# ToyotaResearchInstitute/conex

Hardware: AMD Instinct MI355X
Metric: Newton KKT-solves/sec (assemble+factor+solve), 1000x(20x20) PSD blocks, fp64 (higher is better)
Workload: dtype f64

## Files before the change

### conex_amd/csrc/kkt_context.hip

```cpp
#include <hip/hip_ext.h>
#include "kkt_internal.h"
#include "kernels_cone.hip.h"
#include "kernels_gemm.hip.h"
#include "kernels_kkt_big.hip.h"
#include "kernels_oct.hip.h"
#include "kernels_lmi.hip.h"
#include "lmi_fused_mfma.h"
#include "kernels_lmi_sparse.hip.h"
#include "kernels_lmi_rows.hip.h"
#include "kernels_lmi_large.hip.h"
#include "kernels_quad.hip.h"


namespace cxk_host {

int Fail(cxk_context* ctx, const char* msg) {
  ctx->err = msg;
  fprintf(stderr, "conex_kkt_hip: %s\n", msg);
  return CXK_FAILURE;
}

bool IsUnique(int N, int m, const int* x) {
  std::vector<char> seen(N > 0 ? N : 1, 0);
  for (int i = 0; i < m; i++) {
// ... 889 lines not shown
    CXK_CHAIN(24, 0, 24, 0)
    CXK_CHAIN(24, 8, 24, 8)
    CXK_CHAIN(32, 16, 32, 16)
    CXK_CHAIN(8, 8, 24, 0)
    CXK_CHAIN(16, 8, 24, 0)
    CXK_CHAIN(8, 8, 16, 8)
    CXK_CHAIN(24, 0, 24, 8)
    CXK_CHAIN(24, 0, 32, 16)
#undef CXK_CHAIN
    CXK_DEMAND(done, "internal error: no tree_chain_lean instance for the chain's shapes");
    CXK_TRY(hipGetLastError());
  return CXK_SUCCESS;
}

int MakeFusedTreeArgs(cxk_context* ctx, FusedTreeArgs* out) {
  if (*ctx->fx_flag != 0.0) {
    CXK_TRY(hipStreamSynchronize(ctx->stream));
    CXK_TRY(hipMemcpy(ctx->fx_hand.p, ctx->fx_hand_init.data(), sizeof(double) * ctx->fx_hand_init.size(), hipMemcpyHostToDevice));
    unsigned long long bits = kFusedSentinel;
    double sent;
    memcpy(&sent, &bits, sizeof(sent));
    std::vector<double> ys(ctx->fx_ysig.n, sent);
    CXK_TRY(hipMemcpy(ctx->fx_ysig.p, ys.data(), sizeof(double) * ys.size(), hipMemcpyHostToDevice));
    if (ctx->fx_done.p) {
      CXK_TRY(hipMemset(ctx->fx_done.p, 0, sizeof(unsigned long long) * ctx->fx_done.n));
      ctx->fx_done_target = 0;
    }
    *ctx->fx_flag = 0.0;
    ctx->timeout_pending = true;
  }
  FusedTreeArgs& a = *out;
  a.rec = ctx->fx_rec.p;
  a.count = (int)ctx->level_sn.size();
  a.G = ctx->G.p;
  a.AWc = ctx->AWc.p;
  a.AQcc = ctx->AQcc.p;
  a.b = ctx->b.p;
  a.AW = ctx->AW.p;
  a.AQc = ctx->AQc.p;
  a.slab = ctx->slab.p;
  a.y = ctx->y.p;
  a.pub = ctx->fx_pub.p;
  a.tg_reg = ctx->tg_reg.p;
  a.xreg = ctx->fx_xreg.p;
  a.xsrc = ctx->fx_xsrc.p;
  a.rsrc = ctx->fx_rsrc.p;
// ... 13 lines not shown
  a.k_from = nullptr;
  a.comb = 0;
  a.form = 0;
  a.sc = ctx->sc.p;
  a.sys_sc = ctx->sys_sc.p;
  a.K = (int)ctx->cons.size();
  a.host_flag = ctx->fx_flag;
  a.up_sleep = 30;
  a.count_up = ctx->fused_shard ? ctx->fused_up : a.count;
  a.x = ctx->xbuf.p;
  a.n_xs = ctx->n_xs;
  a.n_xv = ctx->n_xv;
  a.xg = ctx->fx_xg.p;
  a.as_src = ctx->as_src.p;
  a.xs_pt = ctx->xs_pt.p;
  a.pt_ptr = ctx->pt_ptr.p;
  a.pt_src = ctx->pt_src.p;
  a.xr = ctx->fx_xr.p;
  a.rs_src = ctx->rs_src.p;
  a.pf_ptr = ctx->pf_ptr.p;
  a.pf_src = ctx->pf_src.p;
  a.done = ctx->fx_done.p;
  a.done_target = 0;
  return CXK_SUCCESS;
}

int ShardAllReduce(cxk_context* ctx, double* buf, size_t count, int op);
long ExchangeCount(const cxk_context* ctx);

void RaiseHostWord(void* flag) { *static_cast<double*>(flag) = 1.0; }
int DebugReportTimeout(cxk_context* ctx) {
  CXK_TRY(hipMemcpyAsync(ctx->d_fail.p + 1, &ctx->asm_tag, sizeof(int), hipMemcpyHostToDevice, ctx->stream));
  if (ctx->debug_stream_ordered) {
    CXK_TRY(hipLaunchHostFunc(ctx->stream, RaiseHostWord, ctx->fx_flag));
    return CXK_SUCCESS;
  }
  CXK_TRY(hipStreamSynchronize(ctx->stream));
  *ctx->fx_flag = 1.0;
  return CXK_SUCCESS;
}

int LaunchFusedShard(cxk_context* ctx) {
  const cxk_context::AsmPending ap = ctx->asm_pending;
  ctx->asm_pending.on = false;
  FusedTreeArgs a;
  if (MakeFusedTreeArgs(ctx, &a)) return CXK_FAILURE;
// ... 2244 lines not shown
    if (r > 0 || n == 1) total += ms;
  }
  if (avg_ms) *avg_ms = total / (n > 1 ? n - 1 : 1);
  CXK_TRY(hipMemcpy(C, dC.p, sizeof(double) * nc * batch, hipMemcpyDeviceToHost));
  (void)hipEventDestroy(e0);
  (void)hipEventDestroy(e1);
  return CXK_SUCCESS;
}

int cxk_dense_top_columns(const cxk_context* ctx) {
  if (!ctx || !ctx->finalized) return -1;
  return ctx->top_dense.on ? ctx->top_dense.args.T : 0;
}

int cxk_count_sparse_lmi(const cxk_context* ctx) {
  if (!ctx || !ctx->finalized) return -1;
  int k = 0;
  for (size_t i = 0; i < ctx->cons.size(); i++) k += ctx->cons[i].type == CXK_LMI && ctx->owned[i] && ctx->cons[i].sparse;
  return k;
}

int cxk_fused_assembly(const cxk_context* ctx) { return ctx && ctx->fused_asm ? 1 : 0; }
int cxk_fused_tree(const cxk_context* ctx) { return ctx && ctx->fused_tree ? 1 : 0; }

int cxk_fused_tree_timed_out(cxk_context* ctx) {
  if (!ctx || !ctx->timeout_unreported) return 0;
  ctx->timeout_unreported = false;
  return 1;
}

int cxk_debug_force_fused_timeout(cxk_context* ctx) {
  if (!ctx || !ctx->fx_flag || !ctx->fused_tree) return CXK_FAILURE;
  *ctx->fx_flag = 1.0;
  return CXK_SUCCESS;
}

int cxk_debug_fused_timeout_at(cxk_context* ctx, int launch_index, int which) {
  if (!ctx || !ctx->device_ready || !ctx->fx_flag || !ctx->fused_tree) return CXK_FAILURE;
  const bool stream_ordered = (which & CXK_DEBUG_FUSED_STREAM_ORDERED) != 0;
  which &= ~CXK_DEBUG_FUSED_STREAM_ORDERED;
  if (stream_ordered && which != CXK_DEBUG_FUSED_SHARD_TOP) return CXK_FAILURE;
  if (which != CXK_DEBUG_FUSED_FACTOR && which != CXK_DEBUG_FUSED_SHARD_UP && which != CXK_DEBUG_FUSED_SHARD_TOP)
    return CXK_FAILURE;
  if ((which == CXK_DEBUG_FUSED_FACTOR) != (ctx->world <= 1) || (ctx->world > 1 && !ctx->fused_shard))
    return CXK_FAILURE;
  ctx->debug_timeout_at = launch_index >= 0 ? ctx->fused_launches + launch_index : -1;
// ... 140 lines not shown
```

### conex_amd/csrc/kkt_internal.h

```cpp
#pragma once
#include <hip/hip_runtime.h>
#include <dlfcn.h>
#include <rccl/rccl.h>

#include <algorithm>
#include <atomic>
#include <cfloat>
#include <climits>
#include <cmath>
#include <cstdio>
#include <cstdlib>
#include <cstring>
#include <iterator>
#include <map>
#include <memory>
#include <string>
#include <tuple>
#include <vector>

#include "../../include/conex_kkt_hip.h"
#include "kernels_kkt.hip.h"
#include "kernels_kkt_top.hip.h"
#include "lmi_types.h"
#include "symbolic.h"
// ... 167 lines not shown
  DevBuf<int> rs_var2;
  int64_t as_T2 = 0;
  int rs_N2 = 0;
  struct AsmPending {
    bool on = false;
    int with_rhs = 0;
    double k = 0, bs = 0, cs = 0, cb = 0, cq = 0, cw = 0;
  } asm_pending;
  bool fused_tree = false;
  bool fused_split = false;
  bool fused_sweep = false;
  bool fused_shard = false;
  int fused_up = 0;
  DevBuf<GatherRec> fx_xg;
  DevBuf<ResidRec> fx_xr;
  DevBuf<unsigned long long> fx_done;
  unsigned long long fx_done_target = 0;
  int fused_sa = 0, fused_sb = 0;
  DevBuf<int> fx_rec, fx_xreg;
  DevBuf<long long> fx_xsrc, fx_rsrc;
  DevBuf<int> fx_pub;
  DevBuf<double> fx_hand, fx_ysig;
  std::vector<double> fx_hand_init;
  long long fx_updb_base = 0;
  long long fx_fwd_stride = 0;
  unsigned fused_tgen = 0;
  DevBuf<double> y3;
  bool y3_valid = false;
  double y3_bs = 0, y3_cs = 0;
  bool y_deferred = false;
  bool no_y_deferral = false;
  DevBuf<unsigned long long> y_done;
  unsigned long long y_done_target = 0;
  bool no_triple = false;
  unsigned fused_gen = 0;
  double* fx_flag = nullptr;
  int debug_timeout_at = -1, debug_timeout_site = 0, fused_launches = 0;
  int fused_timeouts = 0;
  bool timeout_pending = false;
  bool timeout_unreported = false;
  long long shard_settled_seq = -1;
  int shard_fused_tag = 0;
  long long collectives = 0, shard_launch_collectives = 0;
  bool debug_stream_ordered = false;
  long long calls = 0, redo_call = -1;
  bool asm_deferred = false;
// ... 94 lines not shown
```

### conex_amd/csrc/kkt_plans.hip

```cpp
#define CXK_DEVICE_FUNCTIONS_ONLY
#include "kkt_internal.h"
#include "big_chol.h"

namespace cxk_host {

void ComputeTreeStructure(cxk_context* ctx) {
  const Layout& L = ctx->lay;
  const int K = ctx->md.K;
  ctx->t_ns.assign(K, 0);
  ctx->t_nsep.assign(K, 0);
  ctx->t_start.assign(K, 0);
  ctx->t_level.assign(K, 0);
  ctx->t_parent.assign(K, -1);
  for (int e = 0; e < K; e++) {
    ctx->t_ns[e] = L.supernode_size[e];
    ctx->t_nsep[e] = (int)L.separators[e].size();
    ctx->t_start[e] = L.supernode_start[e];
    if (ctx->t_nsep[e] > 0) ctx->t_parent[e] = L.var_to_sn[L.separators[e][0]];
  }
  for (int i = 0; i < K; i++) {
    if (ctx->t_ns[i] == 0) continue;
    for (int v : L.separators[i]) {
      const int p = L.var_to_sn[v];
      if (ctx->t_level[p] < ctx->t_level[i] + 1) ctx->t_level[p] = ctx->t_level[i] + 1;
// ... 104 lines not shown
      const int64_t n = ctx->t_ns[e];
      ctx->n_xs += n * (n + 1) / 2 + n * ctx->t_nsep[e];
      ctx->n_xv += (int)n;
    }
}

namespace {

struct PlanSwitches {
  bool no_big_dataflow = getenv("CXK_NO_BIG_DATAFLOW") != nullptr;
  bool debug_levels = getenv("CXK_DEBUG_LEVELS") != nullptr;
  bool no_lean = getenv("CXK_NO_LEAN") != nullptr;
  bool no_ranges = getenv("CXK_NO_RANGES") != nullptr;
  bool keep_top = getenv("CXK_KEEP_TOP") != nullptr;
  bool no_chain = getenv("CXK_NO_CHAIN") != nullptr;
  bool no_back_pairs = getenv("CXK_NO_BACK_PAIRS") != nullptr;
  bool no_fused_asm = getenv("CXK_NO_FUSED_ASM") != nullptr;
  bool no_fused_shard = getenv("CXK_NO_FUSED_SHARD") != nullptr;
  bool no_fused_tree = getenv("CXK_NO_FUSED_TREE") != nullptr;
  bool no_fused_wide = getenv("CXK_NO_FUSED_WIDE") != nullptr;
  bool fused_split = getenv("CXK_FUSED_SPLIT") != nullptr;
  bool fused_level_order = getenv("CXK_FUSED_LEVEL_ORDER") != nullptr;
  bool no_fused_sweep = getenv("CXK_NO_FUSED_SWEEP") != nullptr;
  bool no_top_dense = getenv("CXK_NO_TOP_DENSE") != nullptr;
};

struct Verdict {
  bool ok = true;
  const char* why = nullptr;
  bool check(bool cond, const char* msg) {
    ok = ok && cond;
    if (!ok && !why) why = msg;
    return ok;
  }
  void note(const char* msg) { check(true, msg); }
  int refuse(const PlanSwitches& sw, const char* strategy) const {
    if (sw.debug_levels) fprintf(stderr, "%s not taken: %s\n", strategy, why ? why : "(unnamed check)");
    return CXK_SUCCESS;
  }
};

template <typename Rec>
std::vector<Rec> Flatten(const std::vector<std::vector<int64_t>>& lists, std::vector<int>* ptr, std::vector<int64_t>* src) {
  std::vector<Rec> recs(lists.size());
  ptr->assign(lists.size() + 1, 0);
  for (size_t t = 0; t < lists.size(); t++) {
// ... 714 lines not shown
  std::vector<int> v2;
  for (int pvar = 0; pvar < N; pvar++)
    if (!var_own[pvar]) {
      r2.push_back(rg.rec[pvar]);
      v2.push_back(pvar);
    }
  ctx->as_T2 = (int64_t)g2.size();
  ctx->rs_N2 = (int)v2.size();
  if (g2.empty()) g2.push_back(GatherRec{0, -1, 0, 0});
  if (v2.empty()) {
    r2.push_back(ResidRec{-1, 0, 0});
    v2.push_back(0);
  }
  CXK_TRY(ctx->asm_rec.upload(arecs));
  CXK_TRY(ctx->as_rec2.upload(g2));
  CXK_TRY(ctx->rs_rec2.upload(r2));
  CXK_TRY(ctx->rs_var2.upload(v2));
  ctx->fused_asm = true;
  return CXK_SUCCESS;
}


struct FusedTables {
  std::vector<int> recs, xreg, pub;
  std::vector<long long> xsrc, rsrc;
};

bool FusedTreeShapes(const cxk_context* ctx, const PlanSwitches& sw, const UpdateSlots& u, Verdict& v, int* sa, int* sb) {
  const int nlev = ctx->nlev;
  const std::vector<int>& ns = ctx->t_ns;
  const int cnt_all = (int)ctx->level_sn.size();
  const bool wide_single = v.ok && ctx->world <= 1 && cnt_all == 1 && ctx->md.K >= 1 && ns[ctx->level_sn[0]] > 32 &&
                           ns[ctx->level_sn[0]] <= 64 && ctx->t_nsep[ctx->level_sn[0]] == 0 && !sw.no_fused_wide;
  if (wide_single) {
    *sa = *sb = ((ns[ctx->level_sn[0]] + 7) / 8 * 8) << 8;
    return true;
  }
  std::vector<int> shapes;
  for (int l = 0; l < nlev && v.ok; l++) {
    if (ctx->level_ptr[l + 1] == ctx->level_ptr[l]) continue;
    v.ok = !ctx->level_big[l] && ctx->level_nh[l] == ctx->level_ptr[l + 1] - ctx->level_ptr[l];
    for (auto& sg : ctx->level_segs[l]) {
      v.ok = v.ok && sg.shape != 0 && sg.inl;
      if (std::find(shapes.begin(), shapes.end(), sg.shape) == shapes.end()) shapes.push_back(sg.shape);
    }
    for (int pos = ctx->level_ptr[l]; pos < ctx->level_ptr[l + 1] && v.ok; pos++) {
      const int e = ctx->level_sn[pos];
// ... 125 lines not shown
      }
    v.ok = ft->rsrc.size() < (size_t)INT32_MAX && ft->xreg.size() < (size_t)INT32_MAX;
  }
}

void FusedTreePublished(const cxk_context* ctx, const UpdateSlots& u, const std::vector<int>& pos_of, size_t n_upd,
                        size_t n_updb, Verdict& v, FusedTables* ft) {
  const Layout& L = ctx->lay;
  const int cnt_all = (int)ctx->level_sn.size();
  for (int pos = 0; pos < cnt_all && v.ok; pos++) {
    const int e = ctx->level_sn[pos];
    for (int x : L.separators[e]) v.check(pos_of[L.var_to_sn[x]] > pos, "a consumer at a lower position");
  }
  v.ok = v.ok && n_upd + n_updb + 8 < (size_t)INT32_MAX;
  for (int pos = 0; pos < cnt_all && v.ok; pos++) {
    const int e = ctx->level_sn[pos];
    const int nsep = ctx->t_nsep[e];
    int* w = ft->recs.data() + (size_t)pos * kFusedRecWords;
    w[21] = w[22] = 0;
    w[23] = (int)ft->pub.size();
    for (int64_t t = 0; t < (int64_t)nsep * (nsep + 1) / 2; t++) ft->pub.push_back(u.pub_dst[(size_t)(u.upd_off[e] + t)]);
    for (int c = 0; c < nsep; c++) ft->pub.push_back((int)n_upd + u.pubb_dst[(size_t)(u.updb_off[e] + c)]);
  }
}

void DealOverXcds(const cxk_context* ctx, const std::vector<int>& pos_of, std::vector<int>* recs) {
  const Layout& L = ctx->lay;
  const int cnt_all = (int)ctx->level_sn.size();
  std::vector<std::vector<int>> kids(cnt_all);
  std::vector<int> roots;
  for (int pos = 0; pos < cnt_all; pos++) {
    int par = INT32_MAX;
    for (int v : L.separators[ctx->level_sn[pos]]) par = std::min(par, pos_of[L.var_to_sn[v]]);
    if (par == INT32_MAX)
      roots.push_back(pos);
    else
      kids[par].push_back(pos);
  }
  std::vector<int> dfs, stack(roots.rbegin(), roots.rend());
  dfs.reserve(cnt_all);
  while (!stack.empty()) {
    const int u = stack.back();
    stack.pop_back();
    dfs.push_back(u);
    for (auto it = kids[u].rbegin(); it != kids[u].rend(); ++it) stack.push_back(*it);
  }
// ... 69 lines not shown
  if (!v.ok) return v.refuse(sw, "whole-tree launch");
  ft.xreg.resize(ft.xreg.size() + kPullPad, 0);
  ft.xsrc.resize(ft.xsrc.size() + kPullPad * kFusedExtraMax, -1ll);
  ft.rsrc.resize(ft.rsrc.size() + 64 * kFusedExtraMax, -1ll);
  ft.pub.resize(ft.pub.size() + 64, (int)u.slots);
  const double sent = [] {
    double d;
    const unsigned long long bits = kFusedSentinel;
    memcpy(&d, &bits, sizeof(d));
    return d;
  }();
  const size_t hs = us + 3 * ubs + 8;
  ctx->fx_updb_base = (long long)us;
  ctx->fx_fwd_stride = (long long)ubs;
  ctx->fx_hand_init.assign(2 * hs, 0.0);
  for (size_t t = 0; t + 64 < ft.pub.size(); t++) {
    const int d = ft.pub[t];
    if (d != (int)u.slots && d != (int)us + u.slotsb) {
      ctx->fx_hand_init[d] = ctx->fx_hand_init[hs + d] = sent;
      if ((size_t)d >= us)
        for (size_t q = 1; q < 3; q++) ctx->fx_hand_init[d + q * ubs] = ctx->fx_hand_init[hs + d + q * ubs] = sent;
    }
  }
  if (!split && !sharded && !sw.fused_level_order) DealOverXcds(ctx, pos_of, &ft.recs);
  CXK_TRY(ctx->fx_rec.upload(ft.recs));
  CXK_TRY(ctx->fx_xreg.upload(ft.xreg));
  CXK_TRY(ctx->fx_xsrc.upload(ft.xsrc));
  CXK_TRY(ctx->fx_rsrc.upload(ft.rsrc));
  CXK_TRY(ctx->fx_pub.upload(ft.pub));
  CXK_TRY(ctx->fx_hand.upload(ctx->fx_hand_init));
  CXK_TRY(ctx->fx_ysig.upload(std::vector<double>(6 * (size_t)N, sent)));
  CXK_TRY(ctx->y3.alloc(3 * (size_t)N, true));
  ctx->fused_tgen = 0;
  ctx->y3_valid = false;
  if (!ctx->fx_flag) {
    CXK_TRY(hipHostMalloc(reinterpret_cast<void**>(&ctx->fx_flag), 64, hipHostMallocDefault));
    *ctx->fx_flag = 0.0;
  }
  ctx->fused_sa = sa;
  ctx->fused_sb = sb;
  ctx->fused_gen = 0;
  ctx->fused_tree = true;
  ctx->fused_split = split;
  ctx->fused_shard = sharded;
  ctx->fused_up = cnt_up;
  ctx->fused_sweep = !sharded && !sw.no_fused_sweep;
  if (sw.debug_levels)
    fprintf(stderr, "whole tree in %s: %d supernodes, shapes <%d,%d> <%d,%d>, %zu entries / %zu variables with further sources\n",
            sharded ? "two launches around the exchange (own subtrees up + pack, top + down)" : split ? "two launches (up, down)" : "one launch", cnt_all, sa >> 8, sa & 255, sb >> 8, sb & 255,
            ft.xreg.size() - kPullPad, ft.rsrc.size());
  return CXK_SUCCESS;
}

int PlanTopDense(cxk_context* ctx, const PlanSwitches& sw, const UpdateSlots& u) {
  const Layout& L = ctx->lay;
  const int K = ctx->md.K, N = ctx->md.N, nlev = ctx->nlev;
  const std::vector<int>& ns = ctx->t_ns;
  const std::vector<int>& nsep = ctx->t_nsep;
  const std::vector<int>& start = ctx->t_start;
  ctx->top_dense.on = false;
  ctx->dense_level = nlev;
  Verdict v;
  v.check(ctx->world <= 1 && !ctx->use_ldlt && !sw.no_top_dense, "sharded, LDLT or CXK_NO_TOP_DENSE");
  int dt = -1;
  if (v.ok) {
    int cols = 0, count = 0;
    bool clean = true;
    for (int l = nlev - 1; l >= 0 && clean; l--) {
      if (ctx->level_nh[l] != ctx->level_ptr[l + 1] - ctx->level_ptr[l]) break;
      for (int pos = ctx->level_ptr[l]; pos < ctx->level_ptr[l + 1]; pos++) {
        cols += ns[ctx->level_sn[pos]];
        count++;
      }
// ... 239 lines not shown
```

### conex_amd/csrc/tree_fused.h

```cpp
#pragma once
#include <hip/hip_runtime.h>

#include <cstdint>

namespace cxk {

constexpr unsigned long long kFusedSentinel = 0x7FF4C0DEC0DE5EEDull;

constexpr int kFusedRecWords = 64;
constexpr int kFusedExtraTargets = 128;
constexpr int kFusedExtraSlots = 8;
constexpr int kFusedExtraMax = 64;
constexpr int kFusedMaxSlots = 4096;

struct GatherRec;
struct ResidRec;

struct FusedTreeArgs {
  const int* rec;
  int count;
  const double *G, *AWc, *AQcc, *b;
  double *AW, *AQc;
  double* slab;
  double* y;
// ... 18 lines not shown
  int comb;
  int form;
  const double* k_from;
  const double* sc;
  double* sys_sc;
  int K;
  double* host_flag;
  int up_sleep;
  int count_up;
  double* x;
  long long n_xs;
  int n_xv;
  const GatherRec* xg;
  const int64_t* as_src;
  const int* xs_pt;
  const int* pt_ptr;
  const int64_t* pt_src;
  const ResidRec* xr;
  const int64_t* rs_src;
  const int* pf_ptr;
  const int* pf_src;
  unsigned long long* done;
  unsigned long long done_target;
};

constexpr int FusedRhsLane(int nsmax, int smax) { return (nsmax == 16 && smax == 8) || (nsmax == 24 && smax == 0) ? 24 : -1; }

enum FusedTreeMode { kFusedFull = 0, kFusedSolve = 1, kFusedUp = 2, kFusedForward = 3, kFusedDown = 4,
                     kFusedShardUp = 5, kFusedShardTop = 6, kFusedTriple = 7 };

bool FusedTreeCompiled(int shape_a, int shape_b);
int FusedTreeOccupancy(int shape_a, int shape_b, bool sharded = false);
hipError_t LaunchFusedTree(const FusedTreeArgs& a, int shape_a, int shape_b, int mode, hipStream_t stream,
                           hipEvent_t ev_start = nullptr, hipEvent_t ev_stop = nullptr);

}
```

### conex_amd/csrc/tree_fused.hip

```cpp
#include <hip/hip_runtime.h>
#include <hip/hip_ext.h>

#include <type_traits>

#define CXK_DEVICE_FUNCTIONS_ONLY
#include "kernels_kkt.hip.h"
#include "kernels_kkt_top.hip.h"
#include "tree_fused.h"

namespace cxk {

constexpr int kFusedSpinLimit = 1 << 18;

#ifdef CXK_FUSED_STAMPS
constexpr int kFusedStampWaves = 8192;
__device__ long long g_fused_tree_stamp[kFusedStampWaves * 16];
#define FT_STAMP(i) ft_stamp[i] = __builtin_amdgcn_s_memrealtime()
#define FT_COUNT(i, v) ft_stamp[i] = (v)
#define FT_STAMP_DECL long long ft_stamp[16] = {0, 0, 0, 0, 0, 0, 0, 0, 0, 0, 0, 0, 0, 0, 0, 0}
#define FT_STAMP_FLUSH(level)                                                              \
  do {                                                                                     \
    if ((threadIdx.x & 63) == 0 && blockIdx.x < kFusedStampWaves) {                        \
      ft_stamp[15] = (level);                                                              \
      for (int i_ = 0; i_ < 16; i_++) g_fused_tree_stamp[blockIdx.x * 16 + i_] = ft_stamp[i_]; \
// ... 53 lines not shown
  const SnRec R = DecodeRec(w);
  FT_STAMP(1);
  auto f = [&](int i) { return __builtin_amdgcn_readlane(w, 32 + i); };
  const int ns = R.ns, s = R.nsep;
  const bool is_row = lane < ns;
  const int sc = lane - NSMAX;
  const bool is_sep = sc >= 0 && sc < s;
  double* base = A.slab + R.diag_off;
  const unsigned rel = (unsigned)(R.offd_off - R.diag_off);
  const unsigned o0 = is_row ? (unsigned)lane : (is_sep ? rel + (unsigned)(sc * ns) : 0u);
  const unsigned st = is_row ? (unsigned)ns : 1u;
  const int lim = is_row ? lane + 1 : (is_sep ? ns : 0);
  const int gen = A.gen;
  double* handG = A.hand + (int64_t)gen * A.hand_stride;
  double* handO = A.hand + (int64_t)(gen ^ 1) * A.hand_stride;
  double* ysG = A.ysig + (int64_t)gen * A.ysig_stride;
  double* ysO = A.ysig + (int64_t)(gen ^ 1) * A.ysig_stride;
  double* handT = A.hand + (int64_t)A.tgen * A.hand_stride;
  double* handTO = A.hand + (int64_t)(A.tgen ^ 1) * A.hand_stride;
  double* ysT = A.ysig + (int64_t)A.tgen * A.ysig_stride;
  double* ysTO = A.ysig + (int64_t)(A.tgen ^ 1) * A.ysig_stride;
  const int pub_beg = __builtin_amdgcn_readlane(w, 23);
  const int npairs = s * (s + 1) / 2, nv = npairs + NRHS * s;

  const double* Gk = A.G + (FROM_X ? 0 : Join64(f(0), f(1)));
  const int64_t roff = FROM_X ? 0 : Join64(f(2), f(3));
  const int M = f(4);
  const int q = is_row ? lane : (is_sep ? ns + sc : 0);
  const int mypr = (__builtin_amdgcn_ds_bpermute(4 * (32 + 6 + (q >> 2)), w) >> (8 * (q & 3))) & 255;
  const int myp = mypr == 255 ? 0 : mypr;
  const int has_fill = FROM_X ? 0 : f(5);
  double a[NSMAX + SMAX + NCOL];
  double rv[NRHS];
  double fwx = 0.0;
  if constexpr (FROM_X) {
    const int64_t xsb = Join64(f(0), f(1));
    const double* xd = A.x + xsb;
    const unsigned tri = (unsigned)(ns * (ns + 1) / 2);
#pragma unroll
    for (int j = 0; j < NSMAX; j++) {
      const unsigned dj = (unsigned)(j * ns - j * (j - 1) / 2);
      const unsigned idx = is_row ? dj + (unsigned)(lane - j) : tri + (unsigned)(sc * ns + j);
      a[j] = xd[(j < lim) ? idx : 0u];
    }
  } else {
    const char* gb = reinterpret_cast<const char*>(Gk);
// ... 476 lines not shown
    const double dinv = 1.0 / dg;
#pragma unroll
    for (int k = NSMAX - 1; k >= 0; k--) {
      if (lane == k) ub *= dinv;
      ub = fma(-col[k], ReadLane(ub, k), ub);
      if constexpr (NRHS > 1) {
#pragma unroll
        for (int q = 0; q < NRHS - 1; q++) {
          if (lane == k) ubx[q] *= dinv;
          ubx[q] = fma(-col[k], ReadLane(ubx[q], k), ubx[q]);
        }
      }
      if constexpr (QN > 0) {
        if (cnt > 0) {
#pragma unroll
          for (int qq = 0; qq < QN; qq++) {
            if (lane == k) Mb[qq] *= dinv;
            Mb[qq] = fma(-col[k], ReadLane(Mb[qq], k), Mb[qq]);
          }
        }
      }
    }
  }
  constexpr bool ROW0 = NSMAX <= 16 && QN > 0;
  double vsep = 0.0, vsepx[NRHS > 1 ? NRHS - 1 : 1];
#pragma unroll
  for (int q = 0; q < (NRHS > 1 ? NRHS - 1 : 1); q++) vsepx[q] = 0.0;
  if constexpr (ROW0) {
#pragma unroll
    for (int qq = 0; qq < QN; qq++) {
      Mb[qq] = -Mb[qq];
      asm volatile("" : "+v"(Mb[qq]));
    }
  }
  if constexpr (QN > 0) {
    if (cnt > 0) {
      const int sepw = __builtin_amdgcn_ds_bpermute(4 * (24 + (lane < 8 ? lane : 0)), w);
      const int sidx = lane < cnt ? (sepw & 0x3ffffff) : (R.sep[0] & 0x3ffffff);
      const double* src = ysG + sidx;
      double v;
      double vx[NRHS > 1 ? NRHS - 1 : 1];
      vx[0] = 0.0;
      for (int spin = 0;; spin++) {
        v = LoadAgent(src);
        bool pending = (lane < cnt) & IsSentinel(v);
        if constexpr (NRHS > 1) {
#pragma unroll
          for (int q = 0; q < NRHS - 1; q++) {
            vx[q] = LoadAgent(ysT + (int64_t)(1 + q) * A.y_stride + sidx);
            pending |= (lane < cnt) & IsSentinel(vx[q]);
          }
        }
        if (__ballot(pending) == 0) {
          FT_COUNT(14, spin);
          break;
        }
        if (spin >= kFusedSpinLimit) {
          ReportTimeout(A);
          break;
        }
        __builtin_amdgcn_s_sleep(1);
      }
      v = lane < cnt ? v : 0.0;
      if constexpr (NRHS > 1) {
#pragma unroll
        for (int q = 0; q < NRHS - 1; q++) vx[q] = lane < cnt ? vx[q] : 0.0;
      }
      if constexpr (ROW0) {
        vsep = v;
        if constexpr (NRHS > 1) {
#pragma unroll
          for (int q = 0; q < NRHS - 1; q++) vsepx[q] = vx[q];
        }
      } else {
#pragma unroll
        for (int qq = 0; qq < QN; qq++) yv[qq] = ReadLane(v, qq);
        if constexpr (NRHS > 1) {
#pragma unroll
          for (int q = 0; q < NRHS - 1; q++)
#pragma unroll
            for (int qq = 0; qq < QN; qq++) yvx[q][qq] = ReadLane(vx[q], qq);
        }
      }
    }
  }
  FT_STAMP(5);
  double accx[NRHS > 1 ? NRHS - 1 : 1];
  accx[0] = 0.0;
  double acc = ub;
// ... 25 lines not shown
      for (int q = 0; q < NRHS - 1; q++) {
        accx[q] = ubx[q];
#pragma unroll
        for (int qq = 0; qq < QN; qq++) accx[q] = fma(-Mb[qq], yvx[q][qq], accx[q]);
      }
    } else if constexpr (NRHS > 1) {
#pragma unroll
      for (int q = 0; q < NRHS - 1; q++) accx[q] = ubx[q];
    }
    if constexpr (QN > 0) {
#pragma unroll
      for (int qq = 0; qq < QN; qq++) acc = fma(-Mb[qq], yv[qq], acc);
    }
  }
  if (active) StoreAgent(ysG + R.start + lane, acc);
  if constexpr (NRHS > 1) {
#pragma unroll
    for (int q = 0; q < NRHS - 1; q++)
      if (active) StoreAgent(ysT + (int64_t)(1 + q) * A.y_stride + R.start + lane, accx[q]);
  }
  FT_STAMP(6);
  if constexpr (ROWRHS) {
    if (__ballot(active && !(acc == acc)) != 0 && lane == 0) atomicExch(A.fail + 1, A.tag);
  }
  if (active) {
    if constexpr (NRHS == 3) {
      A.y3[R.start + lane] = acc;
      A.y3[A.y_stride + R.start + lane] = accx[0];
      A.y3[2 * A.y_stride + R.start + lane] = accx[1];
      A.y[R.start + lane] = accx[0] - acc;
      StoreAgent(ysTO + A.y_stride + R.start + lane, SentinelValue());
      StoreAgent(ysTO + 2 * A.y_stride + R.start + lane, SentinelValue());
    } else {
      A.y[R.start + lane] = acc;
    }
    A.AW[R.start + lane] = awv;
    A.AQc[R.start + lane] = aqv;
    StoreAgent(ysO + R.start + lane, SentinelValue());
  }
  if (NSMAX <= 32 && cnt == 0) {
#pragma unroll
    for (int j = 0; j < NSMAX; j++)
      if (j < lim) base[o0 + j * st] = a[j];
  }
  if constexpr (SMAX > 0) {
    if (s > 0) {
// ... 461 lines not shown
```

### conex_amd/kkt.py

```python
import ctypes as C
import os

import numpy as np

LIB_PATH = os.path.join(os.path.dirname(os.path.abspath(__file__)), "lib", "libconex.so")
_LIB = None

c_int_p = C.POINTER(C.c_int)
c_long_p = C.POINTER(C.c_long)
c_double_p = C.POINTER(C.c_double)


def _dp(a):
    return a.ctypes.data_as(c_double_p)


def _ip(a):
    return a.ctypes.data_as(c_int_p)


def _lp(a):
    return a.ctypes.data_as(c_long_p)


# ... 41 lines not shown
    "cxk_take_step": (C.c_int, [C.c_void_p, C.c_int, C.c_double, C.c_double]),
    "cxk_prepare_take_step": (C.c_int, [C.c_void_p, C.c_double, C.c_double, c_double_p, C.POINTER(C.c_int)]),
    "cxk_weighted_slack_eigenvalues": (C.c_int, [C.c_void_p, C.c_double, c_double_p]),
    "cxk_get_slab": (C.c_int, [C.c_void_p, c_double_p]),
    "cxk_set_slab": (C.c_int, [C.c_void_p, c_double_p]),
    "cxk_get_constraint_schur": (C.c_int, [C.c_void_p, C.c_int, c_double_p, c_double_p,
                                           c_double_p, c_double_p]),
    "cxk_get_residuals": (C.c_int, [C.c_void_p, c_double_p, c_double_p, c_double_p]),
    "cxk_exchange_buffer": (C.c_int, [C.c_void_p, C.POINTER(C.c_void_p), c_long_p]),
    "cxk_exchange_download": (C.c_int, [C.c_void_p, c_double_p]),
    "cxk_exchange_upload": (C.c_int, [C.c_void_p, c_double_p]),
    "cxk_kkt_local_async": (C.c_int, [C.c_void_p, C.c_double, C.c_double, C.c_double]),
    "cxk_kkt_finish_async": (C.c_int, [C.c_void_p, C.c_double, C.c_double, C.c_double]),
    "cxk_owns_constraint": (C.c_int, [C.c_void_p, C.c_int]),
    "cxk_get_valid_variables": (C.c_int, [C.c_void_p, C.POINTER(C.c_ubyte)]),
    "cxk_shard_info": (C.c_int, [C.c_void_p, c_int_p, c_int_p, c_long_p]),
    "cxk_assemble_local": (C.c_int, [C.c_void_p]),
    "cxk_finish_assemble": (C.c_int, [C.c_void_p]),
    "cxk_assembly_work": (C.c_int, [C.c_void_p, c_double_p, c_double_p]),
    "cxk_count_sparse_lmi": (C.c_int, [C.c_void_p]),
    "cxk_count_lmi_kernel": (C.c_int, [C.c_void_p, C.c_int]),
    "cxk_fused_assembly": (C.c_int, [C.c_void_p]),
    "cxk_fused_tree": (C.c_int, [C.c_void_p]),
    "cxk_comm_init_rccl_solo": (C.c_int, [C.c_void_p]),
    "cxk_set_reference_identity": (C.c_int, [C.c_void_p, C.c_int]),
    "cxk_set_solver_mode": (C.c_int, [C.c_void_p, C.c_int]),
    "cxk_phase_timers": (C.c_int, [C.c_void_p, C.c_int]),
    "cxk_phase_mark": (C.c_int, [C.c_void_p, C.c_int]),
    "cxk_phase_read": (C.c_int, [C.c_void_p, c_double_p, C.c_int]),
    "cxk_comm_unique_id": (C.c_int, [C.c_void_p]),
    "cxk_comm_init_rccl": (C.c_int, [C.c_void_p, C.c_void_p, C.c_int, C.c_int]),
    "cxk_comm_set_allreduce": (C.c_int, [C.c_void_p, C.c_void_p, C.c_void_p]),
    "cxk_comm_selftest": (C.c_int, [C.c_void_p, C.c_int]),
    "cxk_comm_count": (C.c_int, [C.c_void_p]),
    "cxk_dense_top_columns": (C.c_int, [C.c_void_p]),
    "cxk_factor_async": (C.c_int, [C.c_void_p]),
    "cxk_factor_solve_async": (C.c_int, [C.c_void_p, C.c_double, C.c_double, C.c_double]),
    "cxk_factor_direction_async": (C.c_int, [C.c_void_p, C.c_double, C.c_double, C.c_double]),
    "cxk_factor_status": (C.c_int, [C.c_void_p, C.POINTER(C.c_int)]),
    "cxk_step_scalars_async": (C.c_int, [C.c_void_p]),
    "cxk_device_mu_supported": (C.c_int, [C.c_void_p]),
    "cxk_triple_supported": (C.c_int, [C.c_void_p]),
    "cxk_factor_solve_triple_async": (C.c_int, [C.c_void_p, C.c_double, C.c_double]),
    "cxk_select_mu_async": (C.c_int, [C.c_void_p, C.c_double, C.c_double, C.c_int, C.c_double, C.c_double,
                                      C.c_double]),
    "cxk_newton_direction_device_mu": (C.c_int, [C.c_void_p, C.c_double, C.c_double]),
# ... 460 lines not shown
        class _Arr:
            __cuda_array_interface__ = {"shape": (count,), "typestr": "<f8", "data": (ptr, False),
                                        "version": 2}
        return torch.as_tensor(_Arr(), device="cuda")

    def assemble_local(self):
        self._check(self.L.cxk_assemble_local(self.h), "cxk_assemble_local")

    def finish_assemble(self):
        self._check(self.L.cxk_finish_assemble(self.h), "cxk_finish_assemble")

    def dense_top_columns(self):
        return self.L.cxk_dense_top_columns(self.h)

    def count_sparse_lmi(self):
        return self.L.cxk_count_sparse_lmi(self.h)

    def fused_assembly(self):
        return bool(self.L.cxk_fused_assembly(self.h))

    def fused_tree(self):
        return bool(self.L.cxk_fused_tree(self.h))

    def count_lmi_kernel(self, which):
        return self.L.cxk_count_lmi_kernel(self.h, which)

    def assembly_work(self):
        b = C.c_double()
        f = C.c_double()
        self.L.cxk_assembly_work(self.h, C.byref(b), C.byref(f))
        return b.value, f.value

    def enable_timing(self, on=True):
        self.L.cxk_enable_timing(self.h, int(on))

    def kernel_time(self, reset=True):
        ms = C.c_double()
        n = self.L.cxk_kernel_time(self.h, int(reset), C.byref(ms))
        return n, ms.value

    CLOCKS = {"assembly": 0, "tree": 1, "solve": 2, "query": 3, "prepare": 4, "take": 5}

    def kernel_clock(self, which, reset=True):
        ms = C.c_double()
        n = self.L.cxk_kernel_clock(self.h, self.CLOCKS[which] if isinstance(which, str) else int(which),
                                    int(reset), C.byref(ms))
# ... 42 lines not shown
```

### include/conex_kkt_hip.h

```cpp
#ifndef CONEX_KKT_HIP_H
#define CONEX_KKT_HIP_H

#ifdef __cplusplus
extern "C" {
#endif

typedef struct cxk_context cxk_context;

enum { CXK_SUCCESS = 0, CXK_FAILURE = 1 };

enum {
  CXK_LMI = 0,
  CXK_LINEAR = 1,
  CXK_SOC = 2,
  CXK_STATIC = 3,
  CXK_QUAD = 4,
  CXK_OCT = 5
};

int cxk_create(int num_vars, int device, void* stream, cxk_context** out);
void cxk_destroy(cxk_context* ctx);
const char* cxk_last_error(const cxk_context* ctx);

int cxk_add_lmi(cxk_context* ctx, int n, int m, const double* A ,
// ... 101 lines not shown
int cxk_owns_constraint(const cxk_context* ctx, int i);
int cxk_get_valid_variables(const cxk_context* ctx, unsigned char* mask );
int cxk_shard_info(const cxk_context* ctx, int* cut_level, int* num_levels, long* exchange_count);
int cxk_assemble_local(cxk_context* ctx);
int cxk_finish_assemble(cxk_context* ctx);

int cxk_get_step_info(cxk_context* ctx, double* out2k);

int cxk_line_search(cxk_context* ctx, double dinf_upper_bound, double b_scaling, double c_scaling,
                    double* result);

int cxk_gemm_f64(int device, int ta, int tb, int M, int N, int K, int batch, const double* A,
                 const double* B, double* C, double alpha, double beta, int lower_only, int splits,
                 int reps, double* avg_ms);

int cxk_count_sparse_lmi(const cxk_context* ctx);

int cxk_count_lmi_kernel(const cxk_context* ctx, int which);

int cxk_dense_top_columns(const cxk_context* ctx);

int cxk_fused_assembly(const cxk_context* ctx);
int cxk_fused_tree(const cxk_context* ctx);
int cxk_fused_tree_timed_out(cxk_context* ctx);
int cxk_debug_force_fused_timeout(cxk_context* ctx);
enum { CXK_DEBUG_FUSED_FACTOR = 0, CXK_DEBUG_FUSED_SHARD_UP = 1, CXK_DEBUG_FUSED_SHARD_TOP = 2,
       CXK_DEBUG_FUSED_STREAM_ORDERED = 16 };
int cxk_debug_fused_timeout_at(cxk_context* ctx, int launch_index, int which);

int cxk_assembly_work(const cxk_context* ctx, double* bytes, double* flops);
int cxk_kernel_time(cxk_context* ctx, int reset, double* avg_ms);
enum { CXK_CLOCK_ASSEMBLY = 0, CXK_CLOCK_TREE = 1, CXK_CLOCK_SOLVE = 2, CXK_CLOCK_QUERY = 3,
       CXK_CLOCK_PREPARE = 4, CXK_CLOCK_TAKE = 5, CXK_CLOCK_COUNT = 6 };
int cxk_kernel_clock(cxk_context* ctx, int which, int reset, double* avg_ms);
int cxk_set_iterative_refinement(cxk_context* ctx, int iterations);

int cxk_enable_timing(cxk_context* ctx, int on);

#ifdef __cplusplus
}
#endif
#endif
```

Before: 23070.

## Fold leaf supernodes' backward solve into their parent in the fused tree kernel

After: 23310 (median of 6 runs). No clear change (+1.1%).

```diff
diff --git a/conex_amd/csrc/kkt_context.hip b/conex_amd/csrc/kkt_context.hip
--- a/conex_amd/csrc/kkt_context.hip
+++ b/conex_amd/csrc/kkt_context.hip
@@ -935,6 +935,10 @@
     memcpy(&sent, &bits, sizeof(sent));
     std::vector<double> ys(ctx->fx_ysig.n, sent);
     CXK_TRY(hipMemcpy(ctx->fx_ysig.p, ys.data(), sizeof(double) * ys.size(), hipMemcpyHostToDevice));
+    if (ctx->fused_fold > 0) {
+      std::vector<double> lf(ctx->fx_leaf.n, sent);
+      CXK_TRY(hipMemcpy(ctx->fx_leaf.p, lf.data(), sizeof(double) * lf.size(), hipMemcpyHostToDevice));
+    }
     if (ctx->fx_done.p) {
       CXK_TRY(hipMemset(ctx->fx_done.p, 0, sizeof(unsigned long long) * ctx->fx_done.n));
       ctx->fx_done_target = 0;
@@ -994,6 +998,8 @@
   a.pf_src = ctx->pf_src.p;
   a.done = ctx->fx_done.p;
   a.done_target = 0;
+  a.leaf = ctx->fx_leaf.p;
+  a.fold = ctx->fx_fold.p;
   return CXK_SUCCESS;
 }
 
@@ -3284,6 +3290,7 @@
 
 int cxk_fused_assembly(const cxk_context* ctx) { return ctx && ctx->fused_asm ? 1 : 0; }
 int cxk_fused_tree(const cxk_context* ctx) { return ctx && ctx->fused_tree ? 1 : 0; }
+int cxk_fused_fold(const cxk_context* ctx) { return ctx && ctx->fused_tree ? ctx->fused_fold : 0; }
 
 int cxk_fused_tree_timed_out(cxk_context* ctx) {
   if (!ctx || !ctx->timeout_unreported) return 0;
diff --git a/conex_amd/csrc/kkt_internal.h b/conex_amd/csrc/kkt_internal.h
--- a/conex_amd/csrc/kkt_internal.h
+++ b/conex_amd/csrc/kkt_internal.h
@@ -213,6 +213,9 @@
   DevBuf<int> fx_pub;
   DevBuf<double> fx_hand, fx_ysig;
   std::vector<double> fx_hand_init;
+  DevBuf<double> fx_leaf;
+  DevBuf<int> fx_fold;
+  int fused_fold = 0;
   long long fx_updb_base = 0;
   long long fx_fwd_stride = 0;
   unsigned fused_tgen = 0;
diff --git a/conex_amd/csrc/kkt_plans.hip b/conex_amd/csrc/kkt_plans.hip
--- a/conex_amd/csrc/kkt_plans.hip
+++ b/conex_amd/csrc/kkt_plans.hip
@@ -150,6 +150,7 @@
   bool fused_split = getenv("CXK_FUSED_SPLIT") != nullptr;
   bool fused_level_order = getenv("CXK_FUSED_LEVEL_ORDER") != nullptr;
   bool no_fused_sweep = getenv("CXK_NO_FUSED_SWEEP") != nullptr;
+  bool no_fused_fold = getenv("CXK_NO_FUSED_FOLD") != nullptr;
   bool no_top_dense = getenv("CXK_NO_TOP_DENSE") != nullptr;
 };
 
@@ -910,7 +911,7 @@
 
 
 struct FusedTables {
-  std::vector<int> recs, xreg, pub;
+  std::vector<int> recs, xreg, pub, fold;
   std::vector<long long> xsrc, rsrc;
 };
 
@@ -1082,6 +1083,65 @@
     for (int64_t t = 0; t < (int64_t)nsep * (nsep + 1) / 2; t++) ft->pub.push_back(u.pub_dst[(size_t)(u.upd_off[e] + t)]);
     for (int c = 0; c < nsep; c++) ft->pub.push_back((int)n_upd + u.pubb_dst[(size_t)(u.updb_off[e] + c)]);
   }
+}
+
+int FusedTreeFold(const cxk_context* ctx, const std::vector<int>& pos_of, int sa, int sb, FusedTables* ft) {
+  const Layout& L = ctx->lay;
+  const int cnt_all = (int)ctx->level_sn.size();
+  std::vector<std::vector<int>> kids(cnt_all);
+  for (int pos = 0; pos < cnt_all; pos++) {
+    int par = INT32_MAX;
+    for (int v : L.separators[ctx->level_sn[pos]]) par = std::min(par, pos_of[L.var_to_sn[v]]);
+    if (par != INT32_MAX) kids[par].push_back(pos);
+  }
+  auto shape = [&](const SnRec& r) { return sa == sb || RegisterShape(r.ns, r.nsep) == sa ? sa : sb; };
+  int folded = 0;
+  for (int p = 0; p < cnt_all; p++) {
+    const SnRec& P = ctx->h_recs[p];
+    const int cp = P.bs_end - P.bs_beg;
+    if (cp <= 0 || cp > kFoldSep || P.nsep_inline != cp || (shape(P) >> 8) > 32) continue;
+    int n = 0;
+    const int beg = (int)(ft->fold.size() / kFoldWords);
+    for (int c : kids[p]) {
+      const SnRec& C = ctx->h_recs[c];
+      const int cc = C.bs_end - C.bs_beg;
+      if (n == kFoldKids || !kids[c].empty() || C.ns > kFoldRows || cc <= 0 || cc > kFoldSep || C.nsep_inline != cc ||
+          (shape(C) >> 8) > 32)
+        continue;
+      int map[kFoldSep];
+      bool ok = true;
+      for (int qq = 0; qq < kFoldSep; qq++) {
+        map[qq] = kFoldZero;
+        if (qq >= cc) continue;
+        const int x = C.sep[qq] & 0x3ffffff;
+        if (x >= P.start && x < P.start + P.ns) {
+          map[qq] = x - P.start;
+          continue;
+        }
+        int at = -1;
+        for (int q2 = 0; q2 < cp; q2++)
+          if ((P.sep[q2] & 0x3ffffff) == x) at = q2;
+        if (at < 0) ok = false;
+        map[qq] = kFoldSepAt + (at < 0 ? 0 : at);
+      }
+      if (!ok) continue;
+      const int sh = shape(C);
+      const int judge = FusedRhsLane(sh >> 8, sh & 255) >= 0 ? 1 : 0;
+      int* wc = ft->recs.data() + (size_t)c * kFusedRecWords;
+      wc[21] = folded * kFoldSlots;
+      wc[22] = -1;
+      ft->fold.insert(ft->fold.end(), {folded * kFoldSlots, C.start, C.ns | judge << 8, cc});
+      ft->fold.insert(ft->fold.end(), map, map + kFoldSep);
+      folded++;
+      n++;
+    }
+    if (n > 0) {
+      int* wp = ft->recs.data() + (size_t)p * kFusedRecWords;
+      wp[21] = beg;
+      wp[22] = n;
+    }
+  }
+  return folded;
 }
 
 void DealOverXcds(const cxk_context* ctx, const std::vector<int>& pos_of, std::vector<int>* recs) {
@@ -1197,6 +1257,8 @@
         for (size_t q = 1; q < 3; q++) ctx->fx_hand_init[d + q * ubs] = ctx->fx_hand_init[hs + d + q * ubs] = sent;
     }
   }
+  const int folded = !split && !sharded && !wide_single && !sw.no_fused_fold ? FusedTreeFold(ctx, pos_of, sa, sb, &ft) : 0;
+  ft.fold.resize(ft.fold.size() + kFoldWords, kFoldZero);
   if (!split && !sharded && !sw.fused_level_order) DealOverXcds(ctx, pos_of, &ft.recs);
   CXK_TRY(ctx->fx_rec.upload(ft.recs));
   CXK_TRY(ctx->fx_xreg.upload(ft.xreg));
@@ -1205,6 +1267,9 @@
   CXK_TRY(ctx->fx_pub.upload(ft.pub));
   CXK_TRY(ctx->fx_hand.upload(ctx->fx_hand_init));
   CXK_TRY(ctx->fx_ysig.upload(std::vector<double>(6 * (size_t)N, sent)));
+  CXK_TRY(ctx->fx_fold.upload(ft.fold));
+  CXK_TRY(ctx->fx_leaf.upload(std::vector<double>((size_t)(folded > 0 ? folded : 1) * kFoldSlots, sent)));
+  ctx->fused_fold = folded;
   CXK_TRY(ctx->y3.alloc(3 * (size_t)N, true));
   ctx->fused_tgen = 0;
   ctx->y3_valid = false;
@@ -1221,9 +1286,9 @@
   ctx->fused_up = cnt_up;
   ctx->fused_sweep = !sharded && !sw.no_fused_sweep;
   if (sw.debug_levels)
-    fprintf(stderr, "whole tree in %s: %d supernodes, shapes <%d,%d> <%d,%d>, %zu entries / %zu variables with further sources\n",
+    fprintf(stderr, "whole tree in %s: %d supernodes, shapes <%d,%d> <%d,%d>, %zu entries / %zu variables with further sources, %d leaves finished by their parents\n",
             sharded ? "two launches around the exchange (own subtrees up + pack, top + down)" : split ? "two launches (up, down)" : "one launch", cnt_all, sa >> 8, sa & 255, sb >> 8, sb & 255,
-            ft.xreg.size() - kPullPad, ft.rsrc.size());
+            ft.xreg.size() - kPullPad, ft.rsrc.size(), folded);
   return CXK_SUCCESS;
 }
 
diff --git a/conex_amd/csrc/tree_fused.h b/conex_amd/csrc/tree_fused.h
--- a/conex_amd/csrc/tree_fused.h
+++ b/conex_amd/csrc/tree_fused.h
@@ -64,7 +64,16 @@
   const int* pf_src;
   unsigned long long* done;
   unsigned long long done_target;
+  double* leaf;
+  const int* fold;
 };
+
+constexpr int kFoldRows = 16;
+constexpr int kFoldSep = 8;
+constexpr int kFoldKids = 8;
+constexpr int kFoldSlots = kFoldRows * (3 + kFoldSep);
+constexpr int kFoldWords = 4 + kFoldSep;
+constexpr int kFoldSepAt = 64, kFoldZero = 72;
 
 constexpr int FusedRhsLane(int nsmax, int smax) { return (nsmax == 16 && smax == 8) || (nsmax == 24 && smax == 0) ? 24 : -1; }
 
diff --git a/conex_amd/csrc/tree_fused.hip b/conex_amd/csrc/tree_fused.hip
--- a/conex_amd/csrc/tree_fused.hip
+++ b/conex_amd/csrc/tree_fused.hip
@@ -99,6 +99,8 @@
   double* ysTO = A.ysig + (int64_t)(A.tgen ^ 1) * A.ysig_stride;
   const int pub_beg = __builtin_amdgcn_readlane(w, 23);
   const int npairs = s * (s + 1) / 2, nv = npairs + NRHS * s;
+  constexpr bool FOLD = !UP_ONLY && !FROM_X && NSMAX <= 32;
+  const int fold_n = FOLD ? __builtin_amdgcn_readlane(w, 22) : 0;
 
   const double* Gk = A.G + (FROM_X ? 0 : Join64(f(0), f(1)));
   const int64_t roff = FROM_X ? 0 : Join64(f(2), f(3));
@@ -621,6 +623,34 @@
       }
     }
   }
+  if constexpr (FOLD && QN > 0) {
+    if (fold_n < 0) {
+      double* dst = A.leaf + __builtin_amdgcn_readlane(w, 21) + lane;
+      if (active) {
+        StoreAgent(dst, ub);
+        if constexpr (NRHS > 1) {
+#pragma unroll
+          for (int q = 0; q < NRHS - 1; q++) StoreAgent(dst + kFoldRows * (1 + q), ubx[q]);
+        }
+#pragma unroll
+        for (int qq = 0; qq < QN; qq++)
+          if (qq < cnt) StoreAgent(dst + kFoldRows * (3 + qq), Mb[qq]);
+        A.AW[R.start + lane] = awv;
+        A.AQc[R.start + lane] = aqv;
+      }
+      if constexpr (SMAX > 0) {
+        if (s > 0) {
+#pragma unroll
+          for (int r = 0; r < PR; r++)
+            if (lane + 64 * r < nv) StoreAgent((NRHS > 1 && pdt[r] ? handTO : handO) + pd[r], SentinelValue());
+        }
+      }
+      FT_STAMP(5);
+      FT_STAMP(6);
+      FT_STAMP_FLUSH(f(31));
+      return;
+    }
+  }
   constexpr bool ROW0 = NSMAX <= 16 && QN > 0;
   double vsep = 0.0, vsepx[NRHS > 1 ? NRHS - 1 : 1];
 #pragma unroll
@@ -632,6 +662,69 @@
       asm volatile("" : "+v"(Mb[qq]));
     }
   }
+  constexpr int FP = FOLD && QN > 0 ? kFoldKids / 4 : 0;
+  constexpr int FPA = FP > 0 ? FP : 1;
+  const int nfold = FP > 0 && fold_n > 0 ? fold_n : 0;
+  double fu[FPA][NRHS], fm[FPA][kFoldSep];
+  int fmap[FPA][kFoldSep], fstart[FPA];
+  bool frow[FPA], fjudge[FPA];
+  if constexpr (FP > 0) {
+    if (nfold > 0) {
+      const int fr = lane & 15;
+      int fbase[FP], fcnt[FP];
+#pragma unroll
+      for (int p = 0; p < FP; p++) {
+        const int ci = 4 * p + (lane >> 4);
+        const int* e = A.fold + (int64_t)(__builtin_amdgcn_readlane(w, 21) + (ci < nfold ? ci : 0)) * kFoldWords;
+        fbase[p] = e[0];
+        fstart[p] = e[1];
+        const int nsj = e[2];
+        fcnt[p] = e[3];
+#pragma unroll
+        for (int qq = 0; qq < kFoldSep; qq++) fmap[p][qq] = e[4 + qq];
+        frow[p] = ci < nfold && fr < (nsj & 255);
+        fjudge[p] = (nsj >> 8) != 0;
+      }
+      for (int spin = 0;; spin++) {
+        bool pending = false;
+#pragma unroll
+        for (int p = 0; p < FP; p++) {
+          const double* src = A.leaf + fbase[p] + fr;
+#pragma unroll
+          for (int q = 0; q < NRHS; q++) {
+            fu[p][q] = LoadAgent(src + kFoldRows * q);
+            pending |= frow[p] & IsSentinel(fu[p][q]);
+          }
+#pragma unroll
+          for (int qq = 0; qq < kFoldSep; qq++) {
+            fm[p][qq] = LoadAgent(src + kFoldRows * (3 + qq));
+            pending |= frow[p] & (qq < fcnt[p]) & IsSentinel(fm[p][qq]);
+          }
+        }
+        if (__ballot(pending) == 0) break;
+        if (spin >= kFusedSpinLimit) {
+          ReportTimeout(A);
+          break;
+        }
+        __builtin_amdgcn_s_sleep(1);
+      }
+#pragma unroll
+      for (int p = 0; p < FP; p++) {
+        double* src = A.leaf + fbase[p] + fr;
+#pragma unroll
+        for (int q = 0; q < NRHS; q++)
+          if (frow[p]) StoreAgent(src + kFoldRows * q, SentinelValue());
+#pragma unroll
+        for (int qq = 0; qq < kFoldSep; qq++) {
+          if (frow[p] && qq < fcnt[p]) StoreAgent(src + kFoldRows * (3 + qq), SentinelValue());
+          fm[p][qq] = qq < fcnt[p] ? fm[p][qq] : 0.0;
+        }
+      }
+    }
+  }
+  double ysep = 0.0, ysepx[NRHS > 1 ? NRHS - 1 : 1];
+#pragma unroll
+  for (int q = 0; q < (NRHS > 1 ? NRHS - 1 : 1); q++) ysepx[q] = 0.0;
   if constexpr (QN > 0) {
     if (cnt > 0) {
       const int sepw = __builtin_amdgcn_ds_bpermute(4 * (24 + (lane < 8 ? lane : 0)), w);
@@ -664,6 +757,11 @@
       if constexpr (NRHS > 1) {
 #pragma unroll
         for (int q = 0; q < NRHS - 1; q++) vx[q] = lane < cnt ? vx[q] : 0.0;
+      }
+      ysep = v;
+      if constexpr (NRHS > 1) {
+#pragma unroll
+        for (int q = 0; q < NRHS - 1; q++) ysepx[q] = vx[q];
       }
       if constexpr (ROW0) {
         vsep = v;
@@ -735,6 +833,50 @@
   FT_STAMP(6);
   if constexpr (ROWRHS) {
     if (__ballot(active && !(acc == acc)) != 0 && lane == 0) atomicExch(A.fail + 1, A.tag);
+  }
+  if constexpr (FP > 0) {
+    if (nfold > 0) {
+      constexpr int YS = 80;
+      if (active) {
+        my[lane] = acc;
+        if constexpr (NRHS > 1) {
+#pragma unroll
+          for (int q = 0; q < NRHS - 1; q++) my[YS * (1 + q) + lane] = accx[q];
+        }
+      }
+      if (lane < kFoldSep) {
+        my[kFoldSepAt + lane] = ysep;
+        if constexpr (NRHS > 1) {
+#pragma unroll
+          for (int q = 0; q < NRHS - 1; q++) my[YS * (1 + q) + kFoldSepAt + lane] = ysepx[q];
+        }
+      }
+      if (lane < NRHS) my[YS * lane + kFoldZero] = 0.0;
+      WaveSync();
+#pragma unroll
+      for (int p = 0; p < FP; p++) {
+        double c[NRHS];
+#pragma unroll
+        for (int q = 0; q < NRHS; q++) {
+          c[q] = fu[p][q];
+#pragma unroll
+          for (int qq = 0; qq < kFoldSep; qq++) c[q] = fma(-fm[p][qq], my[YS * q + fmap[p][qq]], c[q]);
+        }
+        const int yi = fstart[p] + (lane & 15);
+        if (frow[p]) {
+          if constexpr (NRHS == 3) {
+            A.y3[yi] = c[0];
+            A.y3[A.y_stride + yi] = c[1];
+            A.y3[2 * A.y_stride + yi] = c[2];
+            A.y[yi] = c[1] - c[0];
+          } else {
+            A.y[yi] = c[0];
+          }
+        }
+        if (__ballot(frow[p] && fjudge[p] && !(c[0] == c[0])) != 0 && lane == 0) atomicExch(A.fail + 1, A.tag);
+      }
+      FT_STAMP(13);
+    }
   }
   if (active) {
     if constexpr (NRHS == 3) {
diff --git a/conex_amd/kkt.py b/conex_amd/kkt.py
--- a/conex_amd/kkt.py
+++ b/conex_amd/kkt.py
@@ -87,6 +87,7 @@
     "cxk_count_lmi_kernel": (C.c_int, [C.c_void_p, C.c_int]),
     "cxk_fused_assembly": (C.c_int, [C.c_void_p]),
     "cxk_fused_tree": (C.c_int, [C.c_void_p]),
+    "cxk_fused_fold": (C.c_int, [C.c_void_p]),
     "cxk_comm_init_rccl_solo": (C.c_int, [C.c_void_p]),
     "cxk_set_reference_identity": (C.c_int, [C.c_void_p, C.c_int]),
     "cxk_set_solver_mode": (C.c_int, [C.c_void_p, C.c_int]),
@@ -593,6 +594,9 @@
     def fused_tree(self):
         return bool(self.L.cxk_fused_tree(self.h))
 
+    def fused_fold(self):
+        return int(self.L.cxk_fused_fold(self.h))
+
     def count_lmi_kernel(self, which):
         return self.L.cxk_count_lmi_kernel(self.h, which)
 
diff --git a/include/conex_kkt_hip.h b/include/conex_kkt_hip.h
--- a/include/conex_kkt_hip.h
+++ b/include/conex_kkt_hip.h
@@ -147,6 +147,7 @@
 
 int cxk_fused_assembly(const cxk_context* ctx);
 int cxk_fused_tree(const cxk_context* ctx);
+int cxk_fused_fold(const cxk_context* ctx);
 int cxk_fused_tree_timed_out(cxk_context* ctx);
 int cxk_debug_force_fused_timeout(cxk_context* ctx);
 enum { CXK_DEBUG_FUSED_FACTOR = 0, CXK_DEBUG_FUSED_SHARD_UP = 1, CXK_DEBUG_FUSED_SHARD_TOP = 2,
```
